# fbreitwieser/krakenuniq

Measured on AMD Instinct MI355X. Metric: Mreads/s (150 bp), higher is better.
Workload: dtype u64

## Files before the change

krakenuniq_amd/csrc/ku_short.hip:

```cpp
#include <cstdlib>
#include <type_traits>

#include "ku_device.h"

#define KS_WAVES 4
#ifndef KS_KCT_LOG2
#define KS_KCT_LOG2 8
#endif
#define KS_FLOOR_EVERY 64u
#define KS_HQ 64
#define KS_PAD 16
#ifdef KU_ABLATION
#define KS_ABL(bit) ((ablate & (bit)) != 0)
#else
#define KS_ABL(bit) false
#endif

template <int ITEMS> struct KsGeom {
  static constexpr int MAXN = 64 * ITEMS;
  static constexpr int NWORDS = (MAXN + 31 + 15) / 16 + 3;
  static constexpr int NCODES = (MAXN + 64) / 16 + 4;
  static constexpr int NAMB = (NWORDS + 1) / 2 + 2;
  static constexpr int NMM = MAXN + 64 + 32;
  static constexpr int TCAP_LOG2 = ITEMS <= 2 ? 8 : (ITEMS <= 4 ? 9 : 10);
  static constexpr int KCT_LOG2 = KS_KCT_LOG2;
  static constexpr int RCT_LOG2 = 6;
};

struct __attribute__((packed, aligned(4))) KsQuad {
  uint32_t x, y, z, w;
};
__device__ __forceinline__ uint64_t ks_quad_key(const KsQuad &q) { return ((uint64_t)q.y << 32) | q.x; }
__device__ __forceinline__ uint4 ks_quad_header(const KsQuad &q) { return make_uint4(q.x, q.y, q.z, q.w); }

__device__ __forceinline__ void ks_wave_sync() {
  __builtin_amdgcn_fence(__ATOMIC_RELEASE, "wavefront");
  __builtin_amdgcn_wave_barrier();
  __builtin_amdgcn_fence(__ATOMIC_ACQUIRE, "wavefront");
}

template <int LOG2>
__device__ __forceinline__ void ks_ct_flush(uint32_t *key, uint32_t *cnt, uint32_t *used, unsigned long long *global,
                                            uint32_t lane, uint32_t *hot = nullptr) {
  ks_wave_sync();
  for (uint32_t i = lane; i < (1u << LOG2); i += 64) {
    uint32_t kk = key[i];
#ifdef KS_DIAG_NOHOT
    if (kk == 1) kk = 0;
#endif
    if (hot && kk == 1) { *hot = cnt[i]; kk = 0; }
    if (kk) atomicAdd(&global[kk - 1], (unsigned long long)cnt[i]);
    key[i] = 0;
    cnt[i] = 0;
  }
  if (lane == 0) *used = 0;
  ks_wave_sync();
}

__device__ __forceinline__ uint32_t ks_bmin4(uint32_t a, uint32_t b) {
  const uint32_t m = ((((a | 0x80808080u) - b) & 0x80808080u) >> 7) * 0xFFu;
  return (b & m) | (a & ~m);
}

#define KS_RCT_SLOT 0x40000000u
__device__ __forceinline__ uint32_t ks_rct_node(uint32_t id, const KuTaxDev &tax) {
  return (id & KS_RCT_SLOT) ? ((id & ~KS_RCT_SLOT) ? tax.slot_node[id & ~KS_RCT_SLOT] : 0u) : id;
}
template <int LOG2>
__device__ __forceinline__ void ks_rct_add(uint32_t *key, uint32_t *cnt, uint32_t *used, uint32_t id, const KuTaxDev &tax,
                                           unsigned long long *global) {
  uint32_t h = (id * 2654435761u) >> (32 - LOG2);
#pragma unroll 1
  for (int probe = 0; probe < 8; ++probe) {
    uint32_t cur = key[h];
    if (cur == 0) { key[h] = id + 1; *used += 1; cur = id + 1; }
    if (cur == id + 1) { cnt[h] += 1; return; }
    h = (h + 1) & ((1u << LOG2) - 1);
  }
  atomicAdd(&global[ks_rct_node(id, tax)], 1ull);
}
template <int LOG2>
__device__ __forceinline__ void ks_rct_flush(uint32_t *key, uint32_t *cnt, uint32_t *used, const KuTaxDev &tax,
                                             unsigned long long *global, uint32_t lane, uint32_t *hot = nullptr) {
  ks_wave_sync();
  for (uint32_t i = lane; i < (1u << LOG2); i += 64) {
    uint32_t kk = key[i];
#ifdef KS_DIAG_NOHOT
    if (kk - 1 == KS_RCT_SLOT) kk = 0;
#endif
    if (hot && kk - 1 == KS_RCT_SLOT) { *hot = cnt[i]; kk = 0; }
    if (kk) atomicAdd(&global[ks_rct_node(kk - 1, tax)], (unsigned long long)cnt[i]);
    key[i] = 0;
    cnt[i] = 0;
  }
  if (lane == 0) *used = 0;
  ks_wave_sync();
}

template <int LOG2, bool TRACK>
__device__ __forceinline__ void ks_tab_add(uint32_t *t_key, uint32_t *t_cnt, uint32_t *n_distinct, uint32_t slot, uint32_t count) {
  uint32_t h = (slot * 2654435761u) >> (32 - LOG2);
  for (;;) {
    uint32_t cur = __hip_atomic_load(&t_key[h], __ATOMIC_RELAXED, __HIP_MEMORY_SCOPE_WORKGROUP);
    if (cur == 0) {
      uint32_t old = atomicCAS(&t_key[h], 0u, slot + 1);
      if (TRACK && old == 0) atomicAdd(n_distinct, 1u);
      cur = old == 0 ? slot + 1 : old;
    }
    if (cur == slot + 1) {
      atomicAdd(&t_cnt[h], count);
      break;
    }
    h = (h + 1) & ((1u << LOG2) - 1);
  }
}

// ... 121 lines not shown
  for (uint32_t pos = lane; pos <= mask; pos += 64) {
    const uint32_t kk = ks_gload(&g_key[pos]);
    if (!kk) continue;
    uint32_t score = 0;
    for (uint32_t i = slot_anc_off[kk - 1], i_end = slot_anc_off[kk]; i < i_end; ++i) {
      const uint32_t s = slot_anc[i];
      uint32_t h = (s * 2654435761u) & mask;
      for (;;) {
        const uint32_t cur = ks_gload(&g_key[h]);
        if (cur == s + 1) { score += ks_gload(&g_cnt[h]) & 0xffffu; break; }
        if (cur == 0) break;
        h = (h + 1) & mask;
      }
    }
    atomicAdd(&g_cnt[pos], score << 16);
    my_max = max(my_max, score);
  }
  my_max = ku_wave_max_u32(my_max);
  __threadfence();
  uint32_t last = 0, res = 0;
  bool firstt = true;
  for (;;) {
    uint32_t my_min = 0xFFFFFFFFu;
    for (uint32_t pos = lane; pos <= mask; pos += 64) {
      const uint32_t kk = ks_gload(&g_key[pos]);
      if (kk && (ks_gload(&g_cnt[pos]) >> 16) == my_max && kk - 1 > last) my_min = min(my_min, kk - 1);
    }
    my_min = ku_wave_min_u32(my_min);
    if (my_min == 0xFFFFFFFFu) break;
    const uint32_t node = slot_node[my_min];
    res = firstt ? node : ku_lca_nodes(node_parent, res, node);
    firstt = false;
    last = my_min;
  }
  for (uint32_t pos = lane; pos <= mask; pos += 64)
    if (ks_gload(&g_key[pos])) { g_key[pos] = 0; g_cnt[pos] = 0; }
  __threadfence();
  return res;
}

template <int ITEMS>
__device__ __forceinline__ uint32_t ks_g_insert_items(unsigned long long *g_key, uint64_t g_mask, const uint32_t (&slot)[ITEMS],
                                                      const uint64_t (&hash)[ITEMS], const bool (&want)[ITEMS], uint32_t *err) {
  unsigned long long key[ITEMS], old[ITEMS];
  uint64_t h[ITEMS];
#pragma unroll
  for (int j = 0; j < ITEMS; ++j) {
    key[j] = ((unsigned long long)(slot[j] + 1) << 32) | ks_encode(hash[j]);
    h[j] = ks_mix(key[j]) & g_mask;
  }
#pragma unroll
  for (int j = 0; j < ITEMS; ++j) old[j] = want[j] ? atomicCAS(&g_key[h[j]], 0ull, key[j]) : key[j];
  uint32_t fresh_n = 0;
#pragma unroll
  for (int j = 0; j < ITEMS; ++j) {
    bool fresh = want[j] && old[j] == 0ull;
    if (want[j] && old[j] != 0ull && old[j] != key[j]) {
      bool placed = false;
      for (uint32_t probe = 1; probe < 4096 && !placed; ++probe) {
        h[j] = (h[j] + 1) & g_mask;
        const unsigned long long o = atomicCAS(&g_key[h[j]], 0ull, key[j]);
        fresh = o == 0ull;
        placed = o == 0ull || o == key[j];
      }
      if (!placed) atomicOr(err, 4u);
    }
    fresh_n += (uint32_t)__popcll(__ballot(fresh));
  }
  return fresh_n;
}

#ifndef KS_OCC2
#define KS_OCC2 6
#endif
#define KS_OCC(ITEMS) ((ITEMS) == 2 ? KS_OCC2 : 4)
template <int ITEMS, bool DO_COUNTS, int KK, int MM, bool WIN, int OUT, bool ROUTE = false>
__global__ __launch_bounds__(64 * KS_WAVES, KS_OCC(ITEMS)) void ku_classify_short_kernel(
    KuDbDev db, KuTaxDev tax, KuCountsDev cnt, const uint8_t *__restrict__ seqs, uint64_t n_bytes,
    const uint64_t *__restrict__ seq_off, const uint32_t *__restrict__ seq_len, uint64_t n_reads,
    uint32_t *__restrict__ calls, uint32_t *__restrict__ taxa, uint32_t ablate, uint32_t floor_every,
    uint32_t *__restrict__ spill, uint32_t spill_cap, KuRunsOut ro, KuSparseFast sf, KuRouteIn rin) {
  using G = KsGeom<ITEMS>;
  constexpr uint32_t TCAP = 1u << G::TCAP_LOG2;
  __shared__ uint32_t s_codes[KS_WAVES][G::NCODES];
  __shared__ uint32_t s_amb[KS_WAVES][G::NAMB];
  __shared__ uint32_t s_mm[KS_WAVES][G::NMM];
  __shared__ uint32_t s_tkey[KS_WAVES][TCAP];
  __shared__ uint32_t s_tcnt[KS_WAVES][TCAP];
  __shared__ uint16_t s_tlist[KS_WAVES][WIN ? (int)TCAP : G::MAXN];
  __shared__ uint32_t s_kk[KS_WAVES][1 << G::KCT_LOG2], s_kc[KS_WAVES][1 << G::KCT_LOG2];
  __shared__ uint32_t s_rk[KS_WAVES][1 << G::RCT_LOG2], s_rc[KS_WAVES][1 << G::RCT_LOG2];
  __shared__ uint2 s_hq[KS_WAVES][DO_COUNTS && !ROUTE ? KS_HQ : 1];
  __shared__ uint32_t s_misc[KS_WAVES][4];

  const uint32_t lane = threadIdx.x & 63u;
  const uint32_t wv = (uint32_t)__builtin_amdgcn_readfirstlane((int)(threadIdx.x >> 6));
  uint32_t *codes = s_codes[wv], *amb = s_amb[wv], *mmv = s_mm[wv];
  uint32_t *t_key = s_tkey[wv], *t_cnt = s_tcnt[wv];
  uint16_t *t_list = s_tlist[wv];
  uint16_t *amb16 = reinterpret_cast<uint16_t *>(amb);
  uint32_t *misc = s_misc[wv];
  const uint32_t k = KK ? (uint32_t)KK : db.k, m = KK ? (uint32_t)MM : db.nt, w = k - m + 1;
  const uint32_t key_shift = ku_key_shift(m);
  const uint32_t *tab = reinterpret_cast<const uint32_t *>(db.table);

  for (uint32_t i = lane; i < TCAP; i += 64) { t_key[i] = 0; t_cnt[i] = 0; }
  if (!ROUTE)
    for (uint32_t i = lane; i < (1u << G::KCT_LOG2); i += 64) { s_kk[wv][i] = 0; s_kc[wv][i] = 0; }
  for (uint32_t i = lane; i < (1u << G::RCT_LOG2); i += 64) { s_rk[wv][i] = 0; s_rc[wv][i] = 0; }
  if (lane < 4) misc[lane] = 0;
  ks_wave_sync();

  const uint64_t n_waves = (uint64_t)gridDim.x * KS_WAVES;
#ifdef KS_STAGGER
  {
    const uint32_t steps = ablate >> 16;
    const uint32_t slot = ((uint32_t)blockIdx.x / 256u) % 6u;
    for (uint32_t i = 0; i < slot * steps; ++i) __builtin_amdgcn_s_sleep(1);
  }
#endif
  uint32_t *g_key = WIN ? spill + ((uint64_t)blockIdx.x * KS_WAVES + wv) * 2ull * spill_cap : nullptr;
  uint32_t *g_cnt = WIN ? g_key + spill_cap : nullptr;
  bool spill_used = false;
  unsigned long long ch_pos = 0, ch_end = 0;
  if (OUT != 0 && ro.pre_base1) {
    ch_pos = ((unsigned long long)(ro.pre_base1 - 1u) + (unsigned long long)blockIdx.x * KS_WAVES + wv) * ro.chunk;
    ch_end = ch_pos + ro.chunk;
  }
  auto runs_room = [&](uint32_t need, uint32_t keep, unsigned long long &keep_base) {
    if (ch_pos + need <= ch_end) return;
    const uint32_t want_min = keep ? 2u * (keep + need) : need;
    const uint32_t want = want_min > ro.chunk ? want_min : ro.chunk;
    unsigned long long b = 0;
    if (lane == 0) b = atomicAdd(ro.counter, (unsigned long long)want);
    b = ((unsigned long long)(uint32_t)__builtin_amdgcn_readfirstlane((int)(uint32_t)(b >> 32)) << 32) |
        (uint32_t)__builtin_amdgcn_readfirstlane((int)(uint32_t)b);
    if (keep) {
      __threadfence();
      for (uint32_t i = lane; i < keep; i += 64) {
        if (keep_base + i < ro.cap && b + i < ro.cap) {
          const uint32_t *src = reinterpret_cast<const uint32_t *>(ro.runs + keep_base + i);
          ro.runs[b + i] = make_uint2(ks_gload(src), ks_gload(src + 1));
        }
      }
      keep_base = b;
    }
    ch_pos = b + keep;
    ch_end = b + want;
  };
  uint32_t sp_fresh = 0;
  uint32_t fl_reads =
      floor_every ? (((uint32_t)blockIdx.x * KS_WAVES + wv) * 40503u >> 8) % floor_every : 0u;
  uint32_t fl_scan = 0;
  uint32_t hq_fill = 0;
  uint2 *hq = s_hq[wv];
#ifdef KS_PREFETCH
  constexpr bool ONE_PASS = (G::NWORDS * 4 + 63) / 64 == 1;
  uint64_t r_first = (uint64_t)blockIdx.x * KS_WAVES + wv;
  uint32_t len_n = r_first < n_reads ? seq_len[r_first] : 0;
  uint64_t off_n = r_first < n_reads ? seq_off[r_first] : 0;
  uint32_t pre0 = 0, pre1 = 0;
  bool pre_ok = false;
  auto prefetch = [&](uint32_t plen, uint64_t poff) {
    const uint32_t b0 = 4 * lane;
    const uint64_t a = poff + b0, a0 = a & ~3ull;
    pre_ok = ONE_PASS && b0 < plen && a0 + 8 <= n_bytes;
    if (pre_ok) {
      const uint32_t *q = reinterpret_cast<const uint32_t *>(seqs + a0);
      pre0 = q[0];
      pre1 = q[1];
    }
  };
  if (r_first < n_reads) prefetch(len_n, off_n);
  uint32_t len_nn = r_first + n_waves < n_reads ? seq_len[r_first + n_waves] : 0;
  uint64_t off_nn = r_first + n_waves < n_reads ? seq_off[r_first + n_waves] : 0;
#endif
#ifndef KS_PREFETCH
  uint32_t len_n = 0;
  uint64_t off_n = 0;
  {
    const uint64_t r0 = (uint64_t)blockIdx.x * KS_WAVES + wv;
    if (r0 < n_reads) { len_n = seq_len[r0]; off_n = seq_off[r0]; }
  }
#endif
  for (uint64_t r = (uint64_t)blockIdx.x * KS_WAVES + wv; r < n_reads; r += n_waves) {
#ifdef KS_PREFETCH
    const uint32_t rlen = len_n;
    const uint64_t roff = off_n;
    const uint32_t cur0 = pre0, cur1 = pre1;
    const bool cur_ok = pre_ok;
    len_n = len_nn;
    off_n = off_nn;
    if (r + n_waves < n_reads) prefetch(len_n, off_n); else pre_ok = false;
    if (r + 2 * n_waves < n_reads) { len_nn = seq_len[r + 2 * n_waves]; off_nn = seq_off[r + 2 * n_waves]; }
#else
    const uint32_t rlen = len_n;
    const uint64_t roff = off_n;
    {
      const uint64_t rn = r + n_waves;
      len_n = rn < n_reads ? seq_len[rn] : 0u;
      off_n = rn < n_reads ? seq_off[rn] : 0ull;
    }
#endif
    const uint32_t n_all = rlen >= k ? rlen - k + 1 : 0;
    uint32_t rd_first = 0, rd_cnt = 0, win0 = 0;
    bool rd_table = false, rd_spill = false;
    uint32_t call_node = 0;
    unsigned long long run_base = 0;
    uint32_t run_n = 0, run_prev = 0;
    bool run_has_prev = false;
    do {
    const uint32_t len = WIN ? min(rlen - win0, (uint32_t)G::MAXN + k - 1) : rlen;
    const uint64_t off = roff + win0;
    const uint32_t n = len >= k ? len - k + 1 : 0;
    if (DO_COUNTS) {
      if (!ROUTE && fl_scan) {
        ks_floor_scan(cnt.registers, cnt.hll_floor, fl_scan - 1u, lane);
        fl_scan = 0;
      }
      if (!ROUTE && misc[0] > (1u << G::KCT_LOG2) / 2) ks_ct_flush<G::KCT_LOG2>(s_kk[wv], s_kc[wv], &misc[0], cnt.n_kmers, lane);
      if (!WIN || win0 == 0)
        if (misc[1] > (1u << G::RCT_LOG2) / 2) ks_rct_flush<G::RCT_LOG2>(s_rk[wv], s_rc[wv], &misc[1], tax, cnt.n_reads, lane);
    }
    uint32_t v[ITEMS];
    bool amb_k[ITEMS];
    uint64_t hh[ITEMS];
#pragma unroll
    for (int j = 0; j < ITEMS; ++j) { v[j] = 0; amb_k[j] = false; hh[j] = 0; }

    if (ROUTE) {
      uint32_t tk[ITEMS], kbv[ITEMS];
#pragma unroll
      for (int j = 0; j < ITEMS; ++j) {
        const uint32_t p = j * 64 + lane;
        tk[j] = p < n ? taxa[off + p] : KU_ROUTE_MISS;
      }
#pragma unroll
      for (int j = 0; j < ITEMS; ++j) {
        amb_k[j] = tk[j] == KU_AMBIG;
        kbv[j] = tk[j] < KU_ROUTE_MISS ? rin.kb[tk[j] >> 5] : 0u;
      }
#pragma unroll
      for (int j = 0; j < ITEMS; ++j) v[j] = tk[j] < KU_ROUTE_MISS ? rin.ret[(uint64_t)kbv[j] + (tk[j] & 31u)] : 0u;
    } else if (n > 0) {
#pragma unroll
      for (uint32_t pl = lane; pl < (uint32_t)((G::NWORDS * 4 + 63) / 64) * 64; pl += 64) {
        const uint32_t b0 = 4 * pl;
        uint32_t c8 = 0, a4 = 0xFu;
        if (b0 < len) {
          const uint64_t a = off + b0;
          const uint64_t a0 = a & ~3ull;
          uint32_t d;
#ifdef KS_PREFETCH
          if (cur_ok && pl == lane && win0 == 0) {
            d = __builtin_amdgcn_alignbyte(cur1, cur0, (uint32_t)(a & 3ull));
          } else
#endif
          if (a0 + 8 <= n_bytes) {
            const uint32_t *q = reinterpret_cast<const uint32_t *>(seqs + a0);
            d = __builtin_amdgcn_alignbyte(q[1], q[0], (uint32_t)(a & 3ull));
          } else {
            d = 0;
            for (uint32_t j = 0; j < 4; ++j) d |= (a + j < n_bytes ? (uint32_t)seqs[a + j] : (uint32_t)'N') << (8 * j);
          }
          ku_pack_dword(d, c8, a4);
          const uint32_t valid = len - b0;
          if (valid < 4) a4 |= (1u << (4 - valid)) - 1u;
        }
        const uint32_t q4 = pl & 3u;
        uint32_t word = c8 << (24 - 8 * q4), ab = a4 << (12 - 4 * q4);
        word |= ku_quad_xor1(word);
        ab |= ku_quad_xor1(ab);
        word |= ku_quad_xor2(word);
        ab |= ku_quad_xor2(ab);
        const uint32_t wi = pl >> 2;
        if (q4 == 0 && wi < (uint32_t)G::NWORDS) {
          codes[wi] = word;
          amb16[wi ^ 1u] = (uint16_t)ab;
        }
      }
      ks_wave_sync();

      const uint32_t P = n + w - 1;
      uint64_t canon[ITEMS];
      bool is_fwd[ITEMS], ok[ITEMS];
      uint32_t pk[ITEMS + 1], wr[ITEMS + 1];
      uint32_t tacc = 0xFFFFFFFFu;
      bool tie = false;
      if (lane < KS_PAD) mmv[P + lane] = (0x03FFFFFFu - lane) << KU_PK_KEYSHIFT;
      const bool tail_round = P > (uint32_t)ITEMS * 64u;
      pk[ITEMS] = 0;
      wr[ITEMS] = (uint32_t)G::NMM - 1u;
#pragma unroll
      for (int j = 0; j <= ITEMS; ++j) {
        if (j == ITEMS && !tail_round) break;
        const uint32_t p = j * 64 + lane;
        wr[j] = p < P ? p : (uint32_t)G::NMM - 1u;
        const uint32_t wi = p >> 4, sh = (p & 15u) * 2;
        const uint32_t c0 = codes[wi], c1 = codes[wi + 1], c2 = codes[wi + 2];
        const uint64_t x = ((((uint64_t)c0 << 32) | c1) << sh >> 32 << 32) | ((((uint64_t)c1 << 32) | c2) << sh >> 32);
        const uint32_t mm = (uint32_t)(x >> (64 - 2 * m));
        const uint32_t mrc = ku_revcomp32(mm, m);
        pk[j] = ku_pk_make((mm < mrc ? mm : mrc) ^ db.xor_mask, key_shift, mm <= mrc);
        if ((m & 1u) == 0) tie |= p < P && mm == mrc;
        mmv[wr[j]] = pk[j];
        if (j < ITEMS) {
          const uint64_t fwd = x >> (64 - 2 * k);
          const uint64_t rc = ku_revcomp64(fwd, k);
          is_fwd[j] = fwd <= rc;
          canon[j] = is_fwd[j] ? fwd : rc;
          const uint32_t ai = p >> 5, as = p & 31u;
          const uint64_t a = (((uint64_t)amb[ai] << 32) | amb[ai + 1]) << as;
          amb_k[j] = p < n && (a >> (64 - k)) != 0;
          ok[j] = p < n && !amb_k[j];
        }
      }
      ks_wave_sync();

      uint32_t key[ITEMS], aoff[ITEMS];
      bool plus[ITEMS];
      if (KS_ABL(64u)) {
#pragma unroll
        for (int j = 0; j < ITEMS; ++j) { key[j] = 0; aoff[j] = 0; plus[j] = true; }
      } else {
        uint32_t blk = 1;
        uint32_t tj[ITEMS + 1];
#pragma unroll
        for (int j = 0; j <= ITEMS; ++j) tj[j] = 0xFFFFFFFFu;
        auto doubling = [&](auto nr_c) {
          constexpr int NR = decltype(nr_c)::value;
#pragma unroll
          for (uint32_t sft = 0; sft < 5; ++sft) {
            const uint32_t st = 1u << sft;
            if (2 * st > w) break;
            uint32_t nb[NR];
#pragma unroll
            for (int j = 0; j < NR; ++j) nb[j] = mmv[j * 64 + lane + st] + (st << 1);
            ks_wave_sync();
#pragma unroll
            for (int j = 0; j < NR; ++j) {
              tj[j] = min(tj[j], (pk[j] ^ nb[j]) - 2u);
              pk[j] = min(pk[j], nb[j]);
              mmv[wr[j]] = pk[j];
            }
            ks_wave_sync();
            blk = 2 * st;
          }
        };
        if (tail_round) doubling(std::integral_constant<int, ITEMS + 1>{});
        else doubling(std::integral_constant<int, ITEMS>{});
        if (w > blk) {
#pragma unroll
          for (int j = 0; j < ITEMS; ++j) {
            const uint32_t nbj = mmv[j * 64 + lane + (w - blk)] + ((w - blk) << 1);
            tj[j] = min(tj[j], (pk[j] ^ nbj) - 2u);
            pk[j] = min(pk[j], nbj);
          }
        }
#pragma unroll
        for (int j = 0; j <= ITEMS; ++j) tacc = min(tacc, j * 64 + lane < P ? tj[j] : 0xFFFFFFFFu);
        tie |= tacc < (1u << KU_PK_KEYSHIFT) - 2u;
#pragma unroll
        for (int j = 0; j < ITEMS; ++j) {
          const uint32_t t = (pk[j] >> 1) & 31u;
          key[j] = pk[j] >> KU_PK_KEYSHIFT;
          aoff[j] = is_fwd[j] ? t : w - 1 - t;
          plus[j] = ((pk[j] & 1u) != 0) == is_fwd[j];
        }
        if (__any(tie)) {
          ks_wave_sync();
#pragma unroll
          for (int j = 0; j <= ITEMS; ++j) {
            const uint32_t p = j * 64 + lane;
            if (p < P) {
              const uint32_t wi = p >> 4, sh = (p & 15u) * 2;
              const uint64_t two = ((uint64_t)codes[wi] << 32) | codes[wi + 1];
              const uint32_t mm = (uint32_t)((two << sh) >> (64 - 2 * m));
              const uint32_t mrc = ku_revcomp32(mm, m);
              mmv[p] = (mm < mrc ? mm : mrc) ^ db.xor_mask;
            }
          }
          ks_wave_sync();
#pragma unroll
          for (int j = 0; j < ITEMS; ++j) {
            const uint32_t p = j * 64 + lane;
            if (ok[j]) {
              uint32_t bin;
              key[j] = ku_anchor_exact(mmv + p, w, key_shift, is_fwd[j], aoff[j], bin);
              const uint32_t q = p + (is_fwd[j] ? aoff[j] : w - 1 - aoff[j]);
              const uint32_t wi = q >> 4, sh = (q & 15u) * 2;
              const uint64_t two = ((uint64_t)codes[wi] << 32) | codes[wi + 1];
              const uint32_t mmf = (uint32_t)((two << sh) >> (64 - 2 * m));
              const uint32_t rcm = ku_revcomp32(mmf, m);
              plus[j] = is_fwd[j] ? (mmf <= rcm) : (rcm <= mmf);
            }
          }
// ... 97 lines not shown
#pragma unroll
        for (int j = 0; j < ITEMS; ++j) {
          if (pick[j]) act[j] = false;
          any |= act[j];
        }
      }

    }

    bool uni = false;
    uint32_t uni_slot = 0;
    uint32_t hit_first = 0;
    if (!KS_ABL(32u)) {
      uint32_t mine = 0;
#pragma unroll
      for (int j = 0; j < ITEMS; ++j)
        if (mine == 0) mine = v[j];
      const unsigned long long bal = __ballot(mine != 0);
      const uint32_t first = bal ? ku_wave_bcast(mine, (uint32_t)__ffsll((long long)bal) - 1) : 0u;
      bool diff = false;
#pragma unroll
      for (int j = 0; j < ITEMS; ++j) diff |= (v[j] != 0 && v[j] != first);
      uni = !__any(diff);
      uni_slot = uni ? first : 0u;
      hit_first = first;
      if (!WIN) {
        if (!uni) {
#pragma unroll
          for (int j = 0; j < ITEMS; ++j)
            if (v[j] != 0) ks_tab_add<G::TCAP_LOG2, false>(t_key, t_cnt, nullptr, v[j], 1u);
          uint32_t *urow_hits = nullptr;
          if (OUT == 2 && DO_COUNTS && !KS_ABL(512u)) urow_hits = sf.u_cnt + (size_t)(sf.unit_of[r] - sf.unit_base) * sf.n_slots;
          call_node = ks_tab_resolve<G::TCAP_LOG2>(t_key, t_cnt, t_list, &misc[2], tax, lane, urow_hits);
        }
      } else if (bal) {
        uint32_t w_hits = 0;
#pragma unroll
        for (int j = 0; j < ITEMS; ++j) w_hits += (uint32_t)__popcll(__ballot(v[j] != 0));
        if (!rd_table && !(uni && (rd_first == 0 || rd_first == first))) {
          if (rd_first && lane == 0) ks_tab_add<G::TCAP_LOG2, true>(t_key, t_cnt, &misc[3], rd_first, rd_cnt);
          rd_table = true;
        }
        if (!rd_table) {
          rd_first = first;
          rd_cnt += w_hits;
        } else {
          ks_wave_sync();
          if (!rd_spill && misc[3] > TCAP - (uint32_t)G::MAXN - 32u) {
            ks_spill_migrate(t_key, t_cnt, TCAP, g_key, g_cnt, spill_cap - 1, !spill_used, lane);
            spill_used = true;
            rd_spill = true;
          }
          if (!rd_spill) {
            if (uni) {
              if (lane == 0) ks_tab_add<G::TCAP_LOG2, true>(t_key, t_cnt, &misc[3], first, w_hits);
            } else {
#pragma unroll
              for (int j = 0; j < ITEMS; ++j)
                if (v[j] != 0) ks_tab_add<G::TCAP_LOG2, true>(t_key, t_cnt, &misc[3], v[j], 1u);
            }
          } else {
            if (uni) {
              if (lane == 0) ks_spill_add(g_key, g_cnt, spill_cap - 1, first, w_hits);
            } else {
#pragma unroll
              for (int j = 0; j < ITEMS; ++j)
                if (v[j] != 0) ks_spill_add(g_key, g_cnt, spill_cap - 1, v[j], 1u);
            }
          }
        }
      }
    }

    const uint32_t uni_code = uni && uni_slot ? tax.slot_taxid[uni_slot] : 0u;
    const bool fl_on = DO_COUNTS && !ROUTE && floor_every != 0 && n > 0;
    uint32_t fl_miss = 0, fl_hit = 0;
    if (fl_on && uni) {
      fl_miss = ks_gload(&cnt.hll_floor[0]);
      fl_hit = ks_gload(&cnt.hll_floor[uni_slot]);
    }

    uint32_t n_hit = 0, n_miss = 0;
    if (DO_COUNTS && !ROUTE && n > 0) {
      uint8_t *reg[ITEMS];
      uint32_t rank[ITEMS], seen[ITEMS], fl[ITEMS];
      if (fl_on && !uni) {
#pragma unroll
        for (int j = 0; j < ITEMS; ++j) fl[j] = ks_gload(&cnt.hll_floor[v[j]]);
      } else {
#pragma unroll
        for (int j = 0; j < ITEMS; ++j) fl[j] = v[j] ? fl_hit : fl_miss;
      }
      bool go[ITEMS];
      unsigned long long gob[ITEMS];
      uint32_t n_go = 0;
#pragma unroll
      for (int j = 0; j < ITEMS; ++j) {
        const bool okc = j * 64 + lane < n && !amb_k[j];
        reg[j] = ku_hll_locate(cnt.registers, okc ? v[j] : 0u, hh[j], rank[j]);
        go[j] = okc && rank[j] > fl[j] && !KS_ABL(2u);
        gob[j] = __ballot(go[j]);
        n_go += (uint32_t)__popcll(gob[j]);
      }
      const bool direct = !fl_on || n_go > KS_HQ / 2;
      if (direct) {
#pragma unroll
        for (int j = 0; j < ITEMS; ++j)
          seen[j] = go[j] ? (uint32_t)*reg[j] : 0xFFu;
      } else {
        if (hq_fill + n_go > KS_HQ) {
          ks_hq_drain(hq, hq_fill, cnt.registers, lane);
          hq_fill = 0;
        }
#pragma unroll
        for (int j = 0; j < ITEMS; ++j) {
          const uint32_t at = hq_fill + __builtin_amdgcn_mbcnt_hi((uint32_t)(gob[j] >> 32), __builtin_amdgcn_mbcnt_lo((uint32_t)gob[j], 0u));
          if (go[j]) hq[at] = make_uint2(v[j], (uint32_t)(hh[j] >> (64 - KU_HLL_P)) | (rank[j] << KU_HLL_P));
          hq_fill += (uint32_t)__popcll(gob[j]);
          seen[j] = 0xFFu;
        }
      }
#pragma unroll
      for (int j = 0; j < ITEMS; ++j) {
        const bool okc = j * 64 + lane < n && !amb_k[j];
        ku_hll_raise(reg[j], seen[j], rank[j]);
        if (uni) {
          n_hit += (uint32_t)__popcll(__ballot(okc && v[j] != 0));
          n_miss += (uint32_t)__popcll(__ballot(okc && v[j] == 0));
        } else if (okc && !KS_ABL(4u)) {
          ku_ct_add<G::KCT_LOG2>(s_kk[wv], s_kc[wv], &misc[0], v[j], 1, cnt.n_kmers);
        }
      }
      if (uni && lane == 0 && !KS_ABL(4u)) {
        if (n_hit) ku_ct_add<G::KCT_LOG2>(s_kk[wv], s_kc[wv], &misc[0], uni_slot, n_hit, cnt.n_kmers);
        if (n_miss) ku_ct_add<G::KCT_LOG2>(s_kk[wv], s_kc[wv], &misc[0], 0u, n_miss, cnt.n_kmers);
      }
      if (fl_on && ((++fl_reads) & 0x7fffffffu) >= floor_every) {
        fl_reads = ~fl_reads & 0x80000000u;
        fl_scan = ((fl_reads >> 31) ? hit_first : 0u) + 1u;
      }
    }

    if (OUT == 2 && DO_COUNTS && n > 0) {
      uint32_t *urow = sf.u_cnt + (size_t)(sf.unit_of[r] - sf.unit_base) * sf.n_slots;
      bool any_miss;
      if (KS_ABL(512u)) {
        any_miss = false;
      } else if (uni) {
        if (lane == 0) {
          if (n_hit) atomicAdd(&urow[uni_slot], n_hit);
          if (n_miss) atomicAdd(&urow[0], n_miss);
        }
        any_miss = n_miss != 0;
      } else if (!WIN && !KS_ABL(32u)) {
        uint32_t nm = 0;
#pragma unroll
        for (int j = 0; j < ITEMS; ++j) nm += (uint32_t)__popcll(__ballot(j * 64 + lane < n && !amb_k[j] && v[j] == 0));
        if (lane == 0 && nm) atomicAdd(&urow[0], nm);
        any_miss = nm != 0;
      } else {
        unsigned long long miss_any = 0;
#pragma unroll
        for (int j = 0; j < ITEMS; ++j) {
          const bool okc = j * 64 + lane < n && !amb_k[j];
          unsigned long long todo = __ballot(okc);
          while (todo) {
            const uint32_t lead = (uint32_t)__ffsll((long long)todo) - 1u;
            const uint32_t s0 = ku_wave_bcast(v[j], lead);
            const unsigned long long same = __ballot(okc && v[j] == s0);
            if (lane == lead) atomicAdd(&urow[s0], (uint32_t)__popcll(same));
            todo &= ~same;
          }
          miss_any |= __ballot(okc && v[j] == 0);
        }
        any_miss = miss_any != 0;
      }
      if (any_miss && sf.dense[0] == 0 && !KS_ABL(256u)) {
        bool want[ITEMS];
#pragma unroll
        for (int j = 0; j < ITEMS; ++j) want[j] = j * 64 + lane < n && !amb_k[j] && v[j] == 0;
        sp_fresh += ks_g_insert_items<ITEMS>(sf.g_key, sf.g_mask, v, hh, want, sf.err);
      }
    }

    uint32_t tcode[ITEMS];
    if (uni) {
#pragma unroll
      for (int j = 0; j < ITEMS; ++j) tcode[j] = v[j] ? uni_code : 0u;
    } else {
#pragma unroll
      for (int j = 0; j < ITEMS; ++j) tcode[j] = tax.slot_taxid[v[j]];
    }
    if (OUT == 0) {
#pragma unroll
      for (int j = 0; j < ITEMS; ++j) {
        const uint32_t p = j * 64 + lane;
        if (p < n && !KS_ABL(8u)) taxa[off + p] = amb_k[j] ? KU_AMBIG : tcode[j];
      }
    } else {
      unsigned long long sm[ITEMS];
      uint32_t carry = run_prev, w_runs = 0;
#pragma unroll
      for (int j = 0; j < ITEMS; ++j) {
        tcode[j] = amb_k[j] ? KU_AMBIG : tcode[j];
        uint32_t up = ku_wave_up1(tcode[j]);
        if (lane == 0) up = carry;
        const bool first = j == 0 && lane == 0 && !run_has_prev;
        sm[j] = __ballot(j * 64 + lane < n && (tcode[j] != up || first));
        w_runs += (uint32_t)__popcll(sm[j]);
        carry = (uint32_t)__builtin_amdgcn_readlane((int)tcode[j], 63);
      }
      if (!WIN || run_n == 0) {
        unsigned long long none = 0;
        runs_room(w_runs, 0u, none);
        run_base = ch_pos;
      } else {
        runs_room(w_runs, run_n, run_base);
      }
      uint32_t before = 0;
#pragma unroll
      for (int j = 0; j < ITEMS; ++j) {
        const unsigned long long at = ch_pos + before + (uint32_t)__popcll(sm[j] & ((1ull << lane) - 1ull));
        if (((sm[j] >> lane) & 1ull) && at < ro.cap) ro.runs[at] = make_uint2(tcode[j], win0 + j * 64 + lane);
        before += (uint32_t)__popcll(sm[j]);
      }
      ch_pos += w_runs;
      run_n += w_runs;
      run_prev = carry;
      run_has_prev = true;
    }
    if (!WIN) {
      if (OUT != 0 && lane == 0) {
        ro.run_off[r] = run_base;
        ro.run_cnt[r] = run_n;
      }
      if (lane == 0) {
        calls[r] = uni ? uni_code : tax.node_taxid[call_node];
        if (DO_COUNTS) ks_rct_add<G::RCT_LOG2>(s_rk[wv], s_rc[wv], &misc[1], uni ? (KS_RCT_SLOT | uni_slot) : call_node, tax, cnt.n_reads);
      }
      ks_wave_sync();
      break;
    }
    uint32_t nxt = win0 + (uint32_t)G::MAXN;
    if (!ROUTE && nxt < n_all) {
      uint32_t last1 = 0;
      if (lane < (uint32_t)G::NAMB) {
        const uint32_t lo = 32u * lane;
        uint32_t wd = lo < len ? amb[lane] : 0u;
        if (len - lo < 32u && lo < len) wd &= ~0u << (32u - (len - lo));
        if (wd) last1 = lo + 32u - (uint32_t)__builtin_ctz(wd);
      }
      last1 = ku_wave_max_u32(last1);
      if (last1 > (uint32_t)G::MAXN) {
        const uint32_t skip_to = min(win0 + last1, n_all);
        if (OUT == 0) {
          if (nxt + lane < skip_to) taxa[roff + nxt + lane] = KU_AMBIG;
        } else if (skip_to > nxt && run_prev != KU_AMBIG) {
          runs_room(1u, run_n, run_base);
          if (lane == 0 && ch_pos < ro.cap) ro.runs[ch_pos] = make_uint2(KU_AMBIG, nxt);
          ch_pos += 1;
          run_n += 1;
          run_prev = KU_AMBIG;
        }
        nxt = skip_to;
      }
    }
    ks_wave_sync();
    win0 = nxt;
    } while (win0 < n_all);
    if (WIN) {
      uint32_t code;
      if (!rd_table) code = rd_first ? tax.slot_taxid[rd_first] : 0u;
      else {
        call_node = rd_spill ? ks_spill_resolve(g_key, g_cnt, spill_cap - 1, tax.slot_anc_off, tax.slot_anc, tax.slot_node, tax.node_parent, lane)
                             : ks_tab_resolve<G::TCAP_LOG2>(t_key, t_cnt, t_list, &misc[2], tax, lane);
        if (lane == 0) misc[3] = 0;
        code = tax.node_taxid[call_node];
      }
      if (lane == 0) {
        calls[r] = code;
        if (OUT != 0) {
          ro.run_off[r] = run_base;
          ro.run_cnt[r] = run_n;
        }
        if (DO_COUNTS) ks_rct_add<G::RCT_LOG2>(s_rk[wv], s_rc[wv], &misc[1], rd_table ? call_node : (KS_RCT_SLOT | rd_first), tax, cnt.n_reads);
      }
      ks_wave_sync();
    }
  }
#ifndef KS_DIAG_NOFLUSH
  if (DO_COUNTS) {
    __shared__ uint32_t s_hot[KS_WAVES][2];
    if (lane < 2) s_hot[wv][lane] = 0;
    if (!ROUTE && hq_fill) ks_hq_drain(hq, hq_fill, cnt.registers, lane);
    if (!ROUTE && fl_scan) ks_floor_scan(cnt.registers, cnt.hll_floor, fl_scan - 1u, lane);
    if (!ROUTE) ks_ct_flush<G::KCT_LOG2>(s_kk[wv], s_kc[wv], &misc[0], cnt.n_kmers, lane, &s_hot[wv][0]);
    ks_rct_flush<G::RCT_LOG2>(s_rk[wv], s_rc[wv], &misc[1], tax, cnt.n_reads, lane, &s_hot[wv][1]);
    __syncthreads();
    if (wv == 0 && lane < 2) {
      unsigned long long sum = 0;
#pragma unroll
      for (int q = 0; q < KS_WAVES; ++q) sum += s_hot[q][lane];
      if (sum) atomicAdd(lane == 0 ? &cnt.n_kmers[0] : &cnt.n_reads[0], sum);
    }
  }
#endif
  if (OUT == 2 && lane == 0 && sp_fresh) atomicAdd(sf.g_count, (unsigned long long)sp_fresh);
}

static uint32_t ks_one_pass_max() { return getenv("KU_SHORT_ONE_PASS_MAX") ? (uint32_t)atoi(getenv("KU_SHORT_ONE_PASS_MAX")) : 192u; }
uint32_t ku_short_max_kmers(const KuDbDev &db) {
  const bool whole = db.bin_lo == 0 && db.bin_hi == (1ull << (2 * db.nt));
  return (db.table && whole) ? ks_one_pass_max() : 0;
}
uint32_t ku_short_max_kmers_windowed(const KuDbDev &db) {
  return ku_short_max_kmers(db) ? 65535u : 0u;
}

static unsigned ks_grid(uint64_t n_reads, int items, int n_cu) {
  const char *oe = getenv("KU_SHORT_BLOCKS_PER_CU");
  const uint64_t per_cu = oe ? (uint64_t)atoi(oe) : (n_reads < 500000 ? 1ull : 2ull) * KS_OCC(items);
  const uint64_t want = (n_reads + KS_WAVES - 1) / KS_WAVES, cap = (uint64_t)n_cu * per_cu;
  return (unsigned)(want < cap ? want : cap);
}
static uint32_t ks_spill_cap(uint32_t max_kmers, uint32_t n_slots) {
  const uint32_t distinct = max_kmers < n_slots ? max_kmers : n_slots;
  uint32_t cap = 1024;
  while (cap < 2 * distinct) cap <<= 1;
  return cap;
}
uint64_t ku_short_workspace_bytes(uint32_t max_kmers, uint32_t n_slots, uint64_t n_reads, int n_cu) {
  if (max_kmers <= ks_one_pass_max()) return 0;
  return (uint64_t)ks_grid(n_reads, 2, n_cu) * KS_WAVES * 2ull * ks_spill_cap(max_kmers, n_slots) * 4ull;
}

uint64_t ku_short_grid_waves(uint64_t n_reads, uint32_t max_kmers, int n_cu) {
  const bool windowed = max_kmers > ks_one_pass_max();
  return (uint64_t)ks_grid(n_reads, max_kmers <= 128 || windowed ? 2 : 3, n_cu) * KS_WAVES;
}

int ku_launch_classify_short(const KuDbDev &db, const KuTaxDev &tax, const KuCountsDev &cnt, const uint8_t *d_seqs,
                             uint64_t n_bytes, const uint64_t *d_seq_off, const uint32_t *d_seq_len, uint64_t n_reads,
                             uint32_t max_kmers, uint32_t flags, uint32_t *d_calls, uint32_t *d_taxa, uint32_t *d_hits,
                             void *d_workspace, uint64_t workspace_bytes, int n_cu, hipStream_t stream,
                             const KuRunsOut *runs_out, const KuSparseFast *sparse) {
  if (n_reads == 0) return KU_OK;
  const bool counts = !(flags & KU_F_NO_COUNTS);
  if (flags & KU_F_KEEP_SLOTS) return KU_EINVAL;
  if (sparse && (!runs_out || !counts)) return KU_EINVAL;
  if (!runs_out && !d_taxa) return KU_EINVAL;
  if (d_hits && hipMemsetAsync(d_hits, 0, n_reads * 4, stream) != hipSuccess) return KU_EHIP;
  const char *ab = getenv("KU_ABLATE");
  const uint32_t ablate = ab ? (uint32_t)atoi(ab) : 0u;
  const char *fe = getenv("KU_HLL_FLOOR_EVERY");
  const uint32_t floor_every = fe ? (uint32_t)(atoi(fe) > 0 ? atoi(fe) : 0) : KS_FLOOR_EVERY;
  const bool windowed = max_kmers > ks_one_pass_max();
  const int items = max_kmers <= 128 || windowed ? 2 : 3;
  const dim3 grid(ks_grid(n_reads, items, n_cu)), block(64 * KS_WAVES);
  uint32_t spill_cap = 0;
  if (windowed) {
    if (max_kmers > 65535u) return KU_EINVAL;
    spill_cap = ks_spill_cap(max_kmers, tax.n_slots);
    if (!d_workspace || workspace_bytes < (uint64_t)grid.x * KS_WAVES * 2ull * spill_cap * 4ull) return KU_EINVAL;
  }
  const KuRunsOut ro = runs_out ? *runs_out : KuRunsOut{};
  const KuSparseFast sf = sparse ? *sparse : KuSparseFast{};
  const int out = sparse ? 2 : (runs_out ? 1 : 0);
#define KS_LAUNCH(I, C, K, M, W, O)                                                                                          \
  hipLaunchKernelGGL((ku_classify_short_kernel<I, C, K, M, W, O>), grid, block, 0, stream, db, tax, cnt, d_seqs, n_bytes,    \
                     d_seq_off, d_seq_len, n_reads, d_calls, d_taxa, ablate, floor_every, (uint32_t *)d_workspace, spill_cap, ro, sf,   \
                     KuRouteIn{})
  const int geo = !counts || db.k != 31 ? 0 : (db.nt == 13 ? 13 : (db.nt == 15 ? 15 : 0));
#define KS_GEO(I, W, O)                                      \
  do {                                                       \
    if (!counts) KS_LAUNCH(I, false, 0, 0, W, (O) == 2 ? 1 : (O)); \
    else if (geo == 13) KS_LAUNCH(I, true, 31, 13, W, O);    \
    else if (geo == 15) KS_LAUNCH(I, true, 31, 15, W, O);    \
    else KS_LAUNCH(I, true, 0, 0, W, O);                     \
  } while (0)
#define KS_OUT(I, W)                  \
  do {                                \
    if (out == 0) KS_GEO(I, W, 0);    \
    else if (out == 1) KS_GEO(I, W, 1); \
    else KS_GEO(I, W, 2);             \
  } while (0)
// ... 43 lines not shown
```

Measured before the change: 597.7.

## Consolidate per-wave LDS into struct, branchless sequence load, defer HLL locate

Per-wave shared arrays are grouped into one struct, and arrays a template variant does not use are sized to zero, which shrinks LDS for ROUTE and no-count variants and may allow higher occupancy. The stage-1 sequence load becomes branchless when the read lies inside the buffer: it clamps the dword index, writes every lane to clamped dump slots, and drops the experimental prefetch and stagger paths. The ambiguity check uses a 32-bit funnel shift instead of a 64-bit shift, and the loop counter uses 32-bit stride and signed-difference compares. HLL register address computation and load now happen only in the direct path, and the pointer for off-lane k-mers is built from key 0. These changes cut branches and address arithmetic but add redundant LDS writes and rely on static_asserts for the dump-slot layout.

After: 611.4 (median of 6 runs). +2.3%, better.

```diff
diff --git a/krakenuniq_amd/csrc/ku_short.hip b/krakenuniq_amd/csrc/ku_short.hip
--- a/krakenuniq_amd/csrc/ku_short.hip
+++ b/krakenuniq_amd/csrc/ku_short.hip
@@ -27,11 +27,28 @@
   static constexpr int RCT_LOG2 = 6;
 };
 
+template <int ITEMS, bool WIN, bool SCAN, bool HQ> struct KsWaveLds {
+  using G = KsGeom<ITEMS>;
+  static constexpr int TCAP = 1 << G::TCAP_LOG2;
+  std::conditional_t<HQ, uint2, uint32_t> hq[HQ ? KS_HQ : 0];
+  uint32_t codes[SCAN ? G::NCODES : 0];
+  uint32_t amb[SCAN ? G::NAMB : 0];
+  uint32_t mm[SCAN ? G::NMM : 0];
+  uint32_t tkey[TCAP];
+  uint32_t tcnt[TCAP];
+  uint32_t kk[SCAN ? 1 << G::KCT_LOG2 : 0], kc[SCAN ? 1 << G::KCT_LOG2 : 0];
+  uint32_t rk[1 << G::RCT_LOG2], rc[1 << G::RCT_LOG2];
+  uint32_t misc[4];
+  uint16_t tlist[WIN ? TCAP : G::MAXN];
+};
+
 struct __attribute__((packed, aligned(4))) KsQuad {
   uint32_t x, y, z, w;
 };
 __device__ __forceinline__ uint64_t ks_quad_key(const KsQuad &q) { return ((uint64_t)q.y << 32) | q.x; }
 __device__ __forceinline__ uint4 ks_quad_header(const KsQuad &q) { return make_uint4(q.x, q.y, q.z, q.w); }
+
+__device__ __forceinline__ bool ks_less64(uint64_t a, uint64_t b) { return (int64_t)(a - b) < 0; }
 
 __device__ __forceinline__ void ks_wave_sync() {
   __builtin_amdgcn_fence(__ATOMIC_RELEASE, "wavefront");
@@ -319,43 +336,29 @@
     uint32_t *__restrict__ spill, uint32_t spill_cap, KuRunsOut ro, KuSparseFast sf, KuRouteIn rin) {
   using G = KsGeom<ITEMS>;
   constexpr uint32_t TCAP = 1u << G::TCAP_LOG2;
-  __shared__ uint32_t s_codes[KS_WAVES][G::NCODES];
-  __shared__ uint32_t s_amb[KS_WAVES][G::NAMB];
-  __shared__ uint32_t s_mm[KS_WAVES][G::NMM];
-  __shared__ uint32_t s_tkey[KS_WAVES][TCAP];
-  __shared__ uint32_t s_tcnt[KS_WAVES][TCAP];
-  __shared__ uint16_t s_tlist[KS_WAVES][WIN ? (int)TCAP : G::MAXN];
-  __shared__ uint32_t s_kk[KS_WAVES][1 << G::KCT_LOG2], s_kc[KS_WAVES][1 << G::KCT_LOG2];
-  __shared__ uint32_t s_rk[KS_WAVES][1 << G::RCT_LOG2], s_rc[KS_WAVES][1 << G::RCT_LOG2];
-  __shared__ uint2 s_hq[KS_WAVES][DO_COUNTS && !ROUTE ? KS_HQ : 1];
-  __shared__ uint32_t s_misc[KS_WAVES][4];
+  using Lds = KsWaveLds<ITEMS, WIN, !ROUTE, DO_COUNTS && !ROUTE>;
+  __shared__ Lds s_w[KS_WAVES];
 
   const uint32_t lane = threadIdx.x & 63u;
   const uint32_t wv = (uint32_t)__builtin_amdgcn_readfirstlane((int)(threadIdx.x >> 6));
-  uint32_t *codes = s_codes[wv], *amb = s_amb[wv], *mmv = s_mm[wv];
-  uint32_t *t_key = s_tkey[wv], *t_cnt = s_tcnt[wv];
-  uint16_t *t_list = s_tlist[wv];
+  Lds &sw = s_w[wv];
+  uint32_t *codes = sw.codes, *amb = sw.amb, *mmv = sw.mm;
+  uint32_t *t_key = sw.tkey, *t_cnt = sw.tcnt;
+  uint16_t *t_list = sw.tlist;
   uint16_t *amb16 = reinterpret_cast<uint16_t *>(amb);
-  uint32_t *misc = s_misc[wv];
+  uint32_t *misc = sw.misc;
   const uint32_t k = KK ? (uint32_t)KK : db.k, m = KK ? (uint32_t)MM : db.nt, w = k - m + 1;
   const uint32_t key_shift = ku_key_shift(m);
   const uint32_t *tab = reinterpret_cast<const uint32_t *>(db.table);
 
   for (uint32_t i = lane; i < TCAP; i += 64) { t_key[i] = 0; t_cnt[i] = 0; }
   if (!ROUTE)
-    for (uint32_t i = lane; i < (1u << G::KCT_LOG2); i += 64) { s_kk[wv][i] = 0; s_kc[wv][i] = 0; }
-  for (uint32_t i = lane; i < (1u << G::RCT_LOG2); i += 64) { s_rk[wv][i] = 0; s_rc[wv][i] = 0; }
+    for (uint32_t i = lane; i < (1u << G::KCT_LOG2); i += 64) { sw.kk[i] = 0; sw.kc[i] = 0; }
+  for (uint32_t i = lane; i < (1u << G::RCT_LOG2); i += 64) { sw.rk[i] = 0; sw.rc[i] = 0; }
   if (lane < 4) misc[lane] = 0;
   ks_wave_sync();
 
-  const uint64_t n_waves = (uint64_t)gridDim.x * KS_WAVES;
-#ifdef KS_STAGGER
-  {
-    const uint32_t steps = ablate >> 16;
-    const uint32_t slot = ((uint32_t)blockIdx.x / 256u) % 6u;
-    for (uint32_t i = 0; i < slot * steps; ++i) __builtin_amdgcn_s_sleep(1);
-  }
-#endif
+  const uint32_t n_waves = gridDim.x * KS_WAVES;
   uint32_t *g_key = WIN ? spill + ((uint64_t)blockIdx.x * KS_WAVES + wv) * 2ull * spill_cap : nullptr;
   uint32_t *g_cnt = WIN ? g_key + spill_cap : nullptr;
   bool spill_used = false;
@@ -390,55 +393,22 @@
       floor_every ? (((uint32_t)blockIdx.x * KS_WAVES + wv) * 40503u >> 8) % floor_every : 0u;
   uint32_t fl_scan = 0;
   uint32_t hq_fill = 0;
-  uint2 *hq = s_hq[wv];
-#ifdef KS_PREFETCH
-  constexpr bool ONE_PASS = (G::NWORDS * 4 + 63) / 64 == 1;
-  uint64_t r_first = (uint64_t)blockIdx.x * KS_WAVES + wv;
-  uint32_t len_n = r_first < n_reads ? seq_len[r_first] : 0;
-  uint64_t off_n = r_first < n_reads ? seq_off[r_first] : 0;
-  uint32_t pre0 = 0, pre1 = 0;
-  bool pre_ok = false;
-  auto prefetch = [&](uint32_t plen, uint64_t poff) {
-    const uint32_t b0 = 4 * lane;
-    const uint64_t a = poff + b0, a0 = a & ~3ull;
-    pre_ok = ONE_PASS && b0 < plen && a0 + 8 <= n_bytes;
-    if (pre_ok) {
-      const uint32_t *q = reinterpret_cast<const uint32_t *>(seqs + a0);
-      pre0 = q[0];
-      pre1 = q[1];
-    }
-  };
-  if (r_first < n_reads) prefetch(len_n, off_n);
-  uint32_t len_nn = r_first + n_waves < n_reads ? seq_len[r_first + n_waves] : 0;
-  uint64_t off_nn = r_first + n_waves < n_reads ? seq_off[r_first + n_waves] : 0;
-#endif
-#ifndef KS_PREFETCH
+  uint2 *hq = reinterpret_cast<uint2 *>(sw.hq);
   uint32_t len_n = 0;
   uint64_t off_n = 0;
   {
     const uint64_t r0 = (uint64_t)blockIdx.x * KS_WAVES + wv;
-    if (r0 < n_reads) { len_n = seq_len[r0]; off_n = seq_off[r0]; }
-  }
-#endif
-  for (uint64_t r = (uint64_t)blockIdx.x * KS_WAVES + wv; r < n_reads; r += n_waves) {
-#ifdef KS_PREFETCH
-    const uint32_t rlen = len_n;
-    const uint64_t roff = off_n;
-    const uint32_t cur0 = pre0, cur1 = pre1;
-    const bool cur_ok = pre_ok;
-    len_n = len_nn;
-    off_n = off_nn;
-    if (r + n_waves < n_reads) prefetch(len_n, off_n); else pre_ok = false;
-    if (r + 2 * n_waves < n_reads) { len_nn = seq_len[r + 2 * n_waves]; off_nn = seq_off[r + 2 * n_waves]; }
-#else
+    if (ks_less64(r0, n_reads)) { len_n = seq_len[r0]; off_n = seq_off[r0]; }
+  }
+  for (uint64_t r = (uint64_t)blockIdx.x * KS_WAVES + wv; ks_less64(r, n_reads); r += n_waves) {
     const uint32_t rlen = len_n;
     const uint64_t roff = off_n;
     {
       const uint64_t rn = r + n_waves;
-      len_n = rn < n_reads ? seq_len[rn] : 0u;
-      off_n = rn < n_reads ? seq_off[rn] : 0ull;
-    }
-#endif
+      const bool more = ks_less64(rn, n_reads);
+      len_n = more ? seq_len[rn] : 0u;
+      off_n = more ? seq_off[rn] : 0ull;
+    }
     const uint32_t n_all = rlen >= k ? rlen - k + 1 : 0;
     uint32_t rd_first = 0, rd_cnt = 0, win0 = 0;
     bool rd_table = false, rd_spill = false;
@@ -455,9 +425,10 @@
         ks_floor_scan(cnt.registers, cnt.hll_floor, fl_scan - 1u, lane);
         fl_scan = 0;
       }
-      if (!ROUTE && misc[0] > (1u << G::KCT_LOG2) / 2) ks_ct_flush<G::KCT_LOG2>(s_kk[wv], s_kc[wv], &misc[0], cnt.n_kmers, lane);
+      const uint32_t fill_k = misc[0], fill_r = misc[1];
+      if (!ROUTE && fill_k > (1u << G::KCT_LOG2) / 2) ks_ct_flush<G::KCT_LOG2>(sw.kk, sw.kc, &misc[0], cnt.n_kmers, lane);
       if (!WIN || win0 == 0)
-        if (misc[1] > (1u << G::RCT_LOG2) / 2) ks_rct_flush<G::RCT_LOG2>(s_rk[wv], s_rc[wv], &misc[1], tax, cnt.n_reads, lane);
+        if (fill_r > (1u << G::RCT_LOG2) / 2) ks_rct_flush<G::RCT_LOG2>(sw.rk, sw.rc, &misc[1], tax, cnt.n_reads, lane);
     }
     uint32_t v[ITEMS];
     bool amb_k[ITEMS];
@@ -480,30 +451,27 @@
 #pragma unroll
       for (int j = 0; j < ITEMS; ++j) v[j] = tk[j] < KU_ROUTE_MISS ? rin.ret[(uint64_t)kbv[j] + (tk[j] & 31u)] : 0u;
     } else if (n > 0) {
-#pragma unroll
-      for (uint32_t pl = lane; pl < (uint32_t)((G::NWORDS * 4 + 63) / 64) * 64; pl += 64) {
+      constexpr uint32_t S1_LANES = (uint32_t)((G::NWORDS * 4 + 63) / 64) * 64;
+      constexpr bool S1_CLAMP = S1_LANES / 4 > (uint32_t)G::NCODES || S1_LANES / 4 > 2u * G::NAMB;
+      static_assert(G::NCODES - 1 >= G::NWORDS && 2 * G::NAMB - 1 >= G::NWORDS + 1, "no dump element behind the code words");
+      const bool text_inside = ks_less64(off + len + 6, n_bytes);
+      const uint32_t *text = reinterpret_cast<const uint32_t *>(seqs + (off & ~3ull));
+      const uint32_t text_sh = (uint32_t)off & 3u, last_dw = (len - 1u) & ~3u;
+#pragma unroll
+      for (uint32_t pl = lane; pl < S1_LANES; pl += 64) {
         const uint32_t b0 = 4 * pl;
+        const uint32_t valid = len - min(b0, len);
         uint32_t c8 = 0, a4 = 0xFu;
-        if (b0 < len) {
+        if (text_inside) {
+          const uint32_t *q = text + (min(b0, last_dw) >> 2);
+          ku_pack_dword(__builtin_amdgcn_alignbyte(q[1], q[0], text_sh), c8, a4);
+        } else if (b0 < len) {
           const uint64_t a = off + b0;
-          const uint64_t a0 = a & ~3ull;
-          uint32_t d;
-#ifdef KS_PREFETCH
-          if (cur_ok && pl == lane && win0 == 0) {
-            d = __builtin_amdgcn_alignbyte(cur1, cur0, (uint32_t)(a & 3ull));
-          } else
-#endif
-          if (a0 + 8 <= n_bytes) {
-            const uint32_t *q = reinterpret_cast<const uint32_t *>(seqs + a0);
-            d = __builtin_amdgcn_alignbyte(q[1], q[0], (uint32_t)(a & 3ull));
-          } else {
-            d = 0;
-            for (uint32_t j = 0; j < 4; ++j) d |= (a + j < n_bytes ? (uint32_t)seqs[a + j] : (uint32_t)'N') << (8 * j);
-          }
+          uint32_t d = 0;
+          for (uint32_t j = 0; j < 4; ++j) d |= (a + j < n_bytes ? (uint32_t)seqs[a + j] : (uint32_t)'N') << (8 * j);
           ku_pack_dword(d, c8, a4);
-          const uint32_t valid = len - b0;
-          if (valid < 4) a4 |= (1u << (4 - valid)) - 1u;
-        }
+        }
+        if (valid < 4) a4 |= (1u << (4 - valid)) - 1u;
         const uint32_t q4 = pl & 3u;
         uint32_t word = c8 << (24 - 8 * q4), ab = a4 << (12 - 4 * q4);
         word |= ku_quad_xor1(word);
@@ -511,10 +479,8 @@
         word |= ku_quad_xor2(word);
         ab |= ku_quad_xor2(ab);
         const uint32_t wi = pl >> 2;
-        if (q4 == 0 && wi < (uint32_t)G::NWORDS) {
-          codes[wi] = word;
-          amb16[wi ^ 1u] = (uint16_t)ab;
-        }
+        codes[S1_CLAMP ? min(wi, (uint32_t)G::NCODES - 1u) : wi] = word;
+        amb16[(S1_CLAMP ? min(wi, 2u * G::NAMB - 1u) : wi) ^ 1u] = (uint16_t)ab;
       }
       ks_wave_sync();
 
@@ -524,7 +490,8 @@
       uint32_t pk[ITEMS + 1], wr[ITEMS + 1];
       uint32_t tacc = 0xFFFFFFFFu;
       bool tie = false;
-      if (lane < KS_PAD) mmv[P + lane] = (0x03FFFFFFu - lane) << KU_PK_KEYSHIFT;
+      static_assert(G::MAXN + 30 + 63 < G::NMM - 1, "the sentinels reach the dump slot");
+      mmv[P + lane] = (0x03FFFFFFu - lane) << KU_PK_KEYSHIFT;
       const bool tail_round = P > (uint32_t)ITEMS * 64u;
       pk[ITEMS] = 0;
       wr[ITEMS] = (uint32_t)G::NMM - 1u;
@@ -547,8 +514,8 @@
           is_fwd[j] = fwd <= rc;
           canon[j] = is_fwd[j] ? fwd : rc;
           const uint32_t ai = p >> 5, as = p & 31u;
-          const uint64_t a = (((uint64_t)amb[ai] << 32) | amb[ai + 1]) << as;
-          amb_k[j] = p < n && (a >> (64 - k)) != 0;
+          const uint32_t a = __funnelshift_l(amb[ai + 1], amb[ai], as);
+          amb_k[j] = p < n && (a >> (32 - k)) != 0;
           ok[j] = p < n && !amb_k[j];
         }
       }
@@ -812,8 +779,7 @@
 
     uint32_t n_hit = 0, n_miss = 0;
     if (DO_COUNTS && !ROUTE && n > 0) {
-      uint8_t *reg[ITEMS];
-      uint32_t rank[ITEMS], seen[ITEMS], fl[ITEMS];
+      uint32_t rank[ITEMS], fl[ITEMS];
       if (fl_on && !uni) {
 #pragma unroll
         for (int j = 0; j < ITEMS; ++j) fl[j] = ks_gload(&cnt.hll_floor[v[j]]);
@@ -827,16 +793,22 @@
 #pragma unroll
       for (int j = 0; j < ITEMS; ++j) {
         const bool okc = j * 64 + lane < n && !amb_k[j];
-        reg[j] = ku_hll_locate(cnt.registers, okc ? v[j] : 0u, hh[j], rank[j]);
+        (void)ku_hll_locate(cnt.registers, 0u, hh[j], rank[j]);
         go[j] = okc && rank[j] > fl[j] && !KS_ABL(2u);
         gob[j] = __ballot(go[j]);
         n_go += (uint32_t)__popcll(gob[j]);
       }
       const bool direct = !fl_on || n_go > KS_HQ / 2;
       if (direct) {
-#pragma unroll
-        for (int j = 0; j < ITEMS; ++j)
+        uint8_t *reg[ITEMS];
+        uint32_t seen[ITEMS];
+#pragma unroll
+        for (int j = 0; j < ITEMS; ++j) {
+          reg[j] = ku_hll_locate(cnt.registers, go[j] ? v[j] : 0u, hh[j], rank[j]);
           seen[j] = go[j] ? (uint32_t)*reg[j] : 0xFFu;
+        }
+#pragma unroll
+        for (int j = 0; j < ITEMS; ++j) ku_hll_raise(reg[j], seen[j], rank[j]);
       } else {
         if (hq_fill + n_go > KS_HQ) {
           ks_hq_drain(hq, hq_fill, cnt.registers, lane);
@@ -847,23 +819,21 @@
           const uint32_t at = hq_fill + __builtin_amdgcn_mbcnt_hi((uint32_t)(gob[j] >> 32), __builtin_amdgcn_mbcnt_lo((uint32_t)gob[j], 0u));
           if (go[j]) hq[at] = make_uint2(v[j], (uint32_t)(hh[j] >> (64 - KU_HLL_P)) | (rank[j] << KU_HLL_P));
           hq_fill += (uint32_t)__popcll(gob[j]);
-          seen[j] = 0xFFu;
         }
       }
 #pragma unroll
       for (int j = 0; j < ITEMS; ++j) {
         const bool okc = j * 64 + lane < n && !amb_k[j];
-        ku_hll_raise(reg[j], seen[j], rank[j]);
         if (uni) {
           n_hit += (uint32_t)__popcll(__ballot(okc && v[j] != 0));
           n_miss += (uint32_t)__popcll(__ballot(okc && v[j] == 0));
         } else if (okc && !KS_ABL(4u)) {
-          ku_ct_add<G::KCT_LOG2>(s_kk[wv], s_kc[wv], &misc[0], v[j], 1, cnt.n_kmers);
+          ku_ct_add<G::KCT_LOG2>(sw.kk, sw.kc, &misc[0], v[j], 1, cnt.n_kmers);
         }
       }
       if (uni && lane == 0 && !KS_ABL(4u)) {
-        if (n_hit) ku_ct_add<G::KCT_LOG2>(s_kk[wv], s_kc[wv], &misc[0], uni_slot, n_hit, cnt.n_kmers);
-        if (n_miss) ku_ct_add<G::KCT_LOG2>(s_kk[wv], s_kc[wv], &misc[0], 0u, n_miss, cnt.n_kmers);
+        if (n_hit) ku_ct_add<G::KCT_LOG2>(sw.kk, sw.kc, &misc[0], uni_slot, n_hit, cnt.n_kmers);
+        if (n_miss) ku_ct_add<G::KCT_LOG2>(sw.kk, sw.kc, &misc[0], 0u, n_miss, cnt.n_kmers);
       }
       if (fl_on && ((++fl_reads) & 0x7fffffffu) >= floor_every) {
         fl_reads = ~fl_reads & 0x80000000u;
@@ -966,7 +936,7 @@
       }
       if (lane == 0) {
         calls[r] = uni ? uni_code : tax.node_taxid[call_node];
-        if (DO_COUNTS) ks_rct_add<G::RCT_LOG2>(s_rk[wv], s_rc[wv], &misc[1], uni ? (KS_RCT_SLOT | uni_slot) : call_node, tax, cnt.n_reads);
+        if (DO_COUNTS) ks_rct_add<G::RCT_LOG2>(sw.rk, sw.rc, &misc[1], uni ? (KS_RCT_SLOT | uni_slot) : call_node, tax, cnt.n_reads);
       }
       ks_wave_sync();
       break;
@@ -1013,24 +983,24 @@
           ro.run_off[r] = run_base;
           ro.run_cnt[r] = run_n;
         }
-        if (DO_COUNTS) ks_rct_add<G::RCT_LOG2>(s_rk[wv], s_rc[wv], &misc[1], rd_table ? call_node : (KS_RCT_SLOT | rd_first), tax, cnt.n_reads);
+        if (DO_COUNTS) ks_rct_add<G::RCT_LOG2>(sw.rk, sw.rc, &misc[1], rd_table ? call_node : (KS_RCT_SLOT | rd_first), tax, cnt.n_reads);
       }
       ks_wave_sync();
     }
   }
 #ifndef KS_DIAG_NOFLUSH
   if (DO_COUNTS) {
-    __shared__ uint32_t s_hot[KS_WAVES][2];
-    if (lane < 2) s_hot[wv][lane] = 0;
+    ks_wave_sync();
+    if (lane < 2) misc[2 + lane] = 0;
     if (!ROUTE && hq_fill) ks_hq_drain(hq, hq_fill, cnt.registers, lane);
     if (!ROUTE && fl_scan) ks_floor_scan(cnt.registers, cnt.hll_floor, fl_scan - 1u, lane);
-    if (!ROUTE) ks_ct_flush<G::KCT_LOG2>(s_kk[wv], s_kc[wv], &misc[0], cnt.n_kmers, lane, &s_hot[wv][0]);
-    ks_rct_flush<G::RCT_LOG2>(s_rk[wv], s_rc[wv], &misc[1], tax, cnt.n_reads, lane, &s_hot[wv][1]);
+    if (!ROUTE) ks_ct_flush<G::KCT_LOG2>(sw.kk, sw.kc, &misc[0], cnt.n_kmers, lane, &misc[2]);
+    ks_rct_flush<G::RCT_LOG2>(sw.rk, sw.rc, &misc[1], tax, cnt.n_reads, lane, &misc[3]);
     __syncthreads();
     if (wv == 0 && lane < 2) {
       unsigned long long sum = 0;
 #pragma unroll
-      for (int q = 0; q < KS_WAVES; ++q) sum += s_hot[q][lane];
+      for (int q = 0; q < KS_WAVES; ++q) sum += s_w[q].misc[2 + lane];
       if (sum) atomicAdd(lane == 0 ? &cnt.n_kmers[0] : &cnt.n_reads[0], sum);
     }
   }
```
